# fanzhongyi/ExploreMultiModal

Measured on AMD Instinct MI355X. Metric: image-text pairs/sec fwd+bwd, VLMo-Base, 1/2/4/8 MI355X; % bf16 MFMA roofline, higher is better.
Workload: dtype bf16

## Files before the change

### exploremultimodal_amd/csrc/elementwise.hip

```cpp
#include "common.h"
#include "vlmo_hip.h"
#include <stdarg.h>
#include <stdio.h>

static thread_local char g_err[512] = "";
void vlmo_set_error(const char* fmt, ...) {
    va_list ap;
    va_start(ap, fmt);
    vsnprintf(g_err, sizeof(g_err), fmt, ap);
    va_end(ap);
}
extern "C" const char* vlmo_last_error(void) { return g_err; }
extern "C" int vlmo_abi_version(void) { return VLMO_ABI_VERSION; }

namespace {

__device__ __forceinline__ float fold_column(const float* __restrict__ ws, int ld, int ncols, int c, int r0, int r1) {
    float a = 0.f;
    if (c < ncols)
        for (int r = r0 + threadIdx.y; r < r1; r += 4) a += ws[(size_t)r * ld + c];
    return a;
}
template <typename T>
__device__ __forceinline__ void colsum8(const T* __restrict__ x, int ld, int ncols, int c8, int r0, int r1, float (&acc)[8]) {
// ... 308 lines not shown
        f32x4 g = *(const f32x4*)(dx + o);
        atype += g;
        if (thresh) {
            const uint64_t bits = drop_bits4(seed, o >> 2);
#pragma unroll
            for (int j = 0; j < 4; ++j) g[j] = drop_keep(bits, j, thresh) ? g[j] * inv_keep : 0.f;
        }
        apos += g;
        if (t > 0) {
            const bool mk = masked && masked[(size_t)b * npatch + t - 1];
            if (mk) amask += g;
            st4<bf16>(dproj + ((size_t)b * npatch + t - 1) * d + c4, mk ? f32x4{0.f, 0.f, 0.f, 0.f} : g);
        }
    }
#pragma unroll
    for (int j = 0; j < 4; ++j) {
        if (dpos) dpos[(size_t)t * d + c4 + j] += apos[j];
        if (dtype_row) atomicAdd(dtype_row + c4 + j, atype[j]);
        if (t == 0 && dcls) dcls[c4 + j] += apos[j];
        if (t > 0 && dmask && masked) atomicAdd(dmask + c4 + j, amask[j]);
    }
}

template <int VPL>
__device__ __forceinline__ void embed_txt_row(int64_t id, int t, int m, int lane, int nv, const float* __restrict__ word,
                                              const float* __restrict__ pos, const float* __restrict__ btype0,
                                              const float* __restrict__ ln_w, const float* __restrict__ ln_b,
                                              const float* __restrict__ type0, float* __restrict__ x,
                                              float* __restrict__ xhat, float* __restrict__ rstd, int d, float eps,
                                              uint32_t thresh, float inv_keep, uint64_t seed) {
    f32x4 v[VPL];
    float s = 0.f;
#pragma unroll
    for (int j = 0; j < VPL; ++j) {
        const int i = lane + 64 * j;
        if (i < nv) {
            v[j] = ((const f32x4*)(word + (size_t)id * d))[i] + ((const f32x4*)btype0)[i] +
                   ((const f32x4*)(pos + (size_t)t * d))[i];
            s += v[j][0] + v[j][1] + v[j][2] + v[j][3];
        } else {
            v[j] = f32x4{0.f, 0.f, 0.f, 0.f};
        }
    }
    const float mu = wave_sum(s) / d;
    float q = 0.f;
#pragma unroll
// ... 65 lines not shown
    }
    __device__ __forceinline__ void spill(float (*red)[VPL * 256], int lane) const {
#pragma unroll
        for (int j = 0; j < VPL; ++j)
#pragma unroll
            for (int k = 0; k < 4; ++k) {
                const int idx = (j * 64 + lane) * 4 + k;
                red[0][idx] = aw[j][k];
                red[1][idx] = ab[j][k];
                red[2][idx] = at[j][k];
                red[3][idx] = ae[j][k];
            }
    }
};

__device__ __forceinline__ int embed_txt_red_index(int c) {
    const int i = c >> 2;
    return ((i >> 6) * 64 + (i & 63)) * 4 + (c & 3);
}

template <int VPL>
__device__ __forceinline__ void embed_txt_row_bwd(int64_t id, int m, int lane, int nv, const float* __restrict__ dx,
                                                  const float* __restrict__ xhat, const float* __restrict__ rstd,
                                                  float* __restrict__ dword, EmbedTxtAcc<VPL>& A, int d, uint32_t thresh,
                                                  float inv_keep, uint64_t seed) {
    const float rs = rstd[m];
    f32x4 g[VPL], xh[VPL];
    float s1 = 0.f, s2 = 0.f;
#pragma unroll
    for (int j = 0; j < VPL; ++j) {
        const int i = lane + 64 * j;
        g[j] = f32x4{0.f, 0.f, 0.f, 0.f};
        xh[j] = g[j];
        if (i < nv) {
            f32x4 gy = ((const f32x4*)(dx + (size_t)m * d))[i];
            A.at[j] += gy;
            if (thresh) {
                const uint64_t bits = drop_bits4(seed, ((uint64_t)m * d >> 2) + i);
#pragma unroll
                for (int k = 0; k < 4; ++k) gy[k] = drop_keep(bits, k, thresh) ? gy[k] * inv_keep : 0.f;
            }
            xh[j] = ((const f32x4*)(xhat + (size_t)m * d))[i];
            A.aw[j] += gy * xh[j];
            A.ab[j] += gy;
            g[j] = gy * A.ww[j];
#pragma unroll
            for (int k = 0; k < 4; ++k) {
                s1 += g[j][k];
                s2 += g[j][k] * xh[j][k];
            }
        }
    }
    const float c1 = wave_sum(s1) / d, c2 = wave_sum(s2) / d;
#pragma unroll
    for (int j = 0; j < VPL; ++j) {
        const int i = lane + 64 * j;
        if (i < nv) {
            const f32x4 de = rs * (g[j] - c1 - xh[j] * c2);
            A.ae[j] += de;
#pragma unroll
            for (int k = 0; k < 4; ++k)
                if (dword && id != 0) atomicAdd(dword + (size_t)id * d + 4 * i + k, de[k]);
        }
    }
}

template <int VPL>
__global__ __launch_bounds__(256) void embed_txt_bwd_kernel(const float* __restrict__ dx, const int64_t* __restrict__ ids,
                                                            const float* __restrict__ xhat, const float* __restrict__ rstd,
                                                            const float* __restrict__ ln_w, float* __restrict__ dword,
                                                            float* __restrict__ dpos, float* __restrict__ dbtype0,
                                                            float* __restrict__ dln_w, float* __restrict__ dln_b,
                                                            float* __restrict__ dtype0, int ntok, int T, int d,
                                                            int rows_per_block, uint32_t thresh, float inv_keep,
                                                            uint64_t seed) {
    __shared__ float red[4][4][VPL * 256];
    const int lane = threadIdx.x & 63, wave = threadIdx.x >> 6, nv = d >> 2;
    EmbedTxtAcc<VPL> A;
    A.init(ln_w, lane, nv);
    const int t = blockIdx.x % T;
    const int b0 = (blockIdx.x / T) * rows_per_block, b1 = min(ntok / T, b0 + rows_per_block);
    for (int bq = b0 + wave; bq < b1; bq += 4) {
        const int m = bq * T + t;
        embed_txt_row_bwd<VPL>(ids[m], m, lane, nv, dx, xhat, rstd, dword, A, d, thresh, inv_keep, seed);
    }
    A.spill(red[wave], lane);
    __syncthreads();
    float* outs[4] = {dln_w, dln_b, dtype0, dbtype0};
    for (int c = threadIdx.x; c < d; c += 256) {
        const int idx = embed_txt_red_index(c);
#pragma unroll
        for (int w = 0; w < 4; ++w)
            if (outs[w]) atomicAdd(outs[w] + c, red[0][w][idx] + red[1][w][idx] + red[2][w][idx] + red[3][w][idx]);
        if (dpos) atomicAdd(dpos + (size_t)t * d + c, red[0][3][idx] + red[1][3][idx] + red[2][3][idx] + red[3][3][idx]);
    }
}

template <int VPL>
__global__ __launch_bounds__(256) void embed_txt_rows_bwd_kernel(const float* __restrict__ dx, const int64_t* __restrict__ ids,
                                                                 const int32_t* __restrict__ off, const float* __restrict__ xhat,
                                                                 const float* __restrict__ rstd, const float* __restrict__ ln_w,
                                                                 float* __restrict__ dword, float* __restrict__ ws, int B, int T,
                                                                 int maxlen, int d, int rows_per_block, uint32_t thresh,
                                                                 float inv_keep, uint64_t seed) {
    __shared__ float red[4][4][VPL * 256];
    const int lane = threadIdx.x & 63, wave = threadIdx.x >> 6, nv = d >> 2;
    EmbedTxtAcc<VPL> A;
    A.init(ln_w, lane, nv);
    const int t = blockIdx.x % maxlen;
    const int b0 = (blockIdx.x / maxlen) * rows_per_block, b1 = min(B, b0 + rows_per_block);
    for (int bq = b0 + wave; bq < b1; bq += 4) {
        const int r0 = off[bq];
        if (t >= off[bq + 1] - r0) continue;
        embed_txt_row_bwd<VPL>(ids[(size_t)bq * T + t], r0 + t, lane, nv, dx, xhat, rstd, dword, A, d, thresh, inv_keep,
                               seed);
    }
    A.spill(red[wave], lane);
    __syncthreads();
    float* row = ws + (size_t)blockIdx.x * 4 * d;
    for (int c = threadIdx.x; c < d; c += 256) {
        const int idx = embed_txt_red_index(c);
#pragma unroll
        for (int w = 0; w < 4; ++w) row[w * d + c] = red[0][w][idx] + red[1][w][idx] + red[2][w][idx] + red[3][w][idx];
    }
}

__global__ __launch_bounds__(256) void embed_txt_fold_kernel(const float* __restrict__ ws, int nrows, int maxlen, int d,
                                                             float* __restrict__ dln_w, float* __restrict__ dln_b,
                                                             float* __restrict__ dtype0, float* __restrict__ dbtype0,
                                                             float* __restrict__ dpos) {
    __shared__ float red[4][4][64];
    const int c = blockIdx.x * 64 + threadIdx.x, ld = 4 * d;
    if (blockIdx.y == 0) {
#pragma unroll
        for (int w = 0; w < 4; ++w) red[w][threadIdx.y][threadIdx.x] = fold_column(ws + w * d, ld, d, c, 0, nrows);
        __syncthreads();
        if (c < d) {
            const int w = threadIdx.y;
            float* out = w == 0 ? dln_w : (w == 1 ? dln_b : (w == 2 ? dtype0 : dbtype0));
            if (out) out[c] += red[w][0][threadIdx.x] + red[w][1][threadIdx.x] + red[w][2][threadIdx.x] + red[w][3][threadIdx.x];
        }
    } else {
        const int t = blockIdx.y - 1;
        red[0][threadIdx.y][threadIdx.x] = fold_column(ws + (size_t)t * ld + 3 * d, maxlen * ld, d, c, 0, nrows / maxlen);
        __syncthreads();
        if (threadIdx.y == 0 && c < d && dpos)
            dpos[(size_t)t * d + c] += red[0][0][threadIdx.x] + red[0][1][threadIdx.x] + red[0][2][threadIdx.x] + red[0][3][threadIdx.x];
    }
}

}

int fold_partials(const VlmoColJob& job, VlmoColJob* fold, hipStream_t stream) {
    if (fold) {
        *fold = job;
        return 0;
    }
    int slices = job.rows >= 64 ? 8 : 1;
    const int rps = (job.rows + slices - 1) / slices;
    slices = (job.rows + rps - 1) / rps;
    hipLaunchKernelGGL(reduce_partials_kernel, dim3((job.ncols + 63) / 64, slices), dim3(64, 4), 0, stream,
                       (const float*)job.src, job.rows, job.ncols, job.out[0], job.n0, job.out[1], rps, job.out[2], job.out[3]);
    VLMO_CHECK_LAUNCH("fold_partials");
    return 0;
}

extern "C" int64_t vlmo_reduce_ws_bytes(int ncols) { return reduce_ws_need(ncols); }

namespace {

// ... 145 lines not shown

extern "C" int vlmo_embed_img_finish(const void* proj, const float* cls_tok, const float* mask_tok, const float* pos,
                                     const float* type_row, const uint8_t* masked_pos, float* x, int B, int npatch,
                                     int d, uint32_t drop_thresh, float inv_keep, uint64_t seed, hipStream_t stream) {
    VLMO_CHECK_ARG(proj && cls_tok && mask_tok && pos && type_row && x, "vlmo_embed_img_finish: null pointer");
    VLMO_CHECK_ARG(B > 0 && npatch > 0 && d % 4 == 0 && d <= 4096, "vlmo_embed_img_finish: bad shape");
    hipLaunchKernelGGL(embed_img_finish_kernel, dim3(npatch + 1, B), dim3(d / 4), 0, stream, (const bf16*)proj, cls_tok,
                       mask_tok, pos, type_row, masked_pos, x, npatch, d, drop_thresh, inv_keep, seed);
    VLMO_CHECK_LAUNCH("vlmo_embed_img_finish");
    return 0;
}

extern "C" int vlmo_embed_img_bwd(const float* dx, const uint8_t* masked_pos, void* dproj, float* dcls, float* dmask,
                                  float* dpos, float* dtype_row, int B, int npatch, int d, uint32_t drop_thresh,
                                  float inv_keep, uint64_t seed, hipStream_t stream) {
    VLMO_CHECK_ARG(dx && dproj, "vlmo_embed_img_bwd: null pointer");
    VLMO_CHECK_ARG(B > 0 && npatch > 0 && d % 4 == 0 && d <= 4096, "vlmo_embed_img_bwd: bad shape");
    hipLaunchKernelGGL(embed_img_bwd_kernel, dim3(npatch + 1), dim3(d / 4), 0, stream, dx, masked_pos, (bf16*)dproj,
                       dcls, dmask, dpos, dtype_row, B, npatch, d, drop_thresh, inv_keep, seed);
    VLMO_CHECK_LAUNCH("vlmo_embed_img_bwd");
    return 0;
}

extern "C" int vlmo_embed_txt_fwd(const int64_t* ids, const float* word, const float* pos, const float* btype0,
                                  const float* ln_w, const float* ln_b, const float* type0, float* x, float* xhat,
                                  float* rstd, int B, int T, int d, float eps, uint32_t drop_thresh, float inv_keep,
                                  uint64_t seed, hipStream_t stream) {
    VLMO_CHECK_ARG(ids && word && pos && btype0 && ln_w && ln_b && type0 && x, "vlmo_embed_txt_fwd: null pointer");
    VLMO_CHECK_ARG(B > 0 && T > 0 && d % 4 == 0 && d <= 1024, "vlmo_embed_txt_fwd: bad shape");
    const int ntok = B * T;
    const int grid = (ntok + 3) / 4 < 8192 ? (ntok + 3) / 4 : 8192;
    dispatch_vpl(d, [&](auto V) {
        hipLaunchKernelGGL(embed_txt_fwd_kernel<decltype(V)::value>, dim3(grid), dim3(256), 0, stream, ids, word, pos, btype0,
                           ln_w, ln_b, type0, x, xhat, rstd, ntok, T, d, eps, drop_thresh, inv_keep, seed);
    });
    VLMO_CHECK_LAUNCH("vlmo_embed_txt_fwd");
    return 0;
}

extern "C" int vlmo_embed_txt_bwd(const float* dx, const int64_t* ids, const float* xhat, const float* rstd,
                                  const float* ln_w, float* dword, float* dpos, float* dbtype0, float* dln_w,
                                  float* dln_b, float* dtype0, int B, int T, int d, uint32_t drop_thresh,
                                  float inv_keep, uint64_t seed, hipStream_t stream) {
    VLMO_CHECK_ARG(dx && ids && xhat && rstd && ln_w, "vlmo_embed_txt_bwd: null pointer");
    VLMO_CHECK_ARG(B > 0 && T > 0 && d % 4 == 0 && d <= 1024, "vlmo_embed_txt_bwd: bad shape");
    const int ntok = B * T;
// ... 30 lines not shown
    if (B <= 0 || maxlen <= 0 || d <= 0) return 0;
    const int rpb = embed_txt_rows_rpb(B);
    return (int64_t)maxlen * ((B + rpb - 1) / rpb) * 4 * d * (int64_t)sizeof(float);
}

extern "C" int vlmo_embed_txt_rows_bwd(const float* dx, const int64_t* ids, const int32_t* off, const float* xhat,
                                       const float* rstd, const float* ln_w, float* dword, float* dpos, float* dbtype0,
                                       float* dln_w, float* dln_b, float* dtype0, float* ws, int64_t ws_bytes, int B, int T,
                                       int maxlen, int d, uint32_t drop_thresh, float inv_keep, uint64_t seed,
                                       hipStream_t stream) {
    VLMO_CHECK_ARG(dx && ids && off && xhat && rstd && ln_w && ws, "vlmo_embed_txt_rows_bwd: null pointer");
    VLMO_CHECK_ARG(B > 0 && T > 0 && maxlen > 0 && maxlen <= T && d % 4 == 0 && d > 0 && d <= 1024,
                   "vlmo_embed_txt_rows_bwd: bad shape B=%d T=%d maxlen=%d d=%d", B, T, maxlen, d);
    VLMO_CHECK_ARG(ws_bytes >= vlmo_embed_txt_rows_ws_bytes(B, maxlen, d),
                   "vlmo_embed_txt_rows_bwd: workspace too small (need %lld bytes)",
                   (long long)vlmo_embed_txt_rows_ws_bytes(B, maxlen, d));
    const int rpb = embed_txt_rows_rpb(B);
    const int grid = maxlen * ((B + rpb - 1) / rpb);
    dispatch_vpl(d, [&](auto V) {
        hipLaunchKernelGGL(embed_txt_rows_bwd_kernel<decltype(V)::value>, dim3(grid), dim3(256), 0, stream, dx, ids, off, xhat,
                           rstd, ln_w, dword, ws, B, T, maxlen, d, rpb, drop_thresh, inv_keep, seed);
    });
    VLMO_CHECK_LAUNCH("vlmo_embed_txt_rows_bwd");
    hipLaunchKernelGGL(embed_txt_fold_kernel, dim3((d + 63) / 64, 1 + maxlen), dim3(64, 4), 0, stream, (const float*)ws, grid,
                       maxlen, d, dln_w, dln_b, dtype0, dbtype0, dpos);
    VLMO_CHECK_LAUNCH("vlmo_embed_txt_rows_bwd");
    return 0;
}
```

### exploremultimodal_amd/engine.py

```python
import ctypes
import functools
import os as _os
import sys
from collections import namedtuple

import torch

from . import hip

LN_EPS = 1e-12
GRAD_SINK = None
_ov = _os.environ.get('VLMO_OVERLAP_WGRAD')
OVERLAP_WGRAD = None if _ov is None else _ov != '0'
ONE_STREAM_ROWS = 12288


def _use_side_stream(sink, rows):
    if OVERLAP_WGRAD is not None:
        return OVERLAP_WGRAD
    return sink is not None or rows < ONE_STREAM_ROWS


DEFAULT_TILE = -1

# ... 51 lines not shown

def _seg(a0, la, b0, lb, device):
    return torch.stack([a0, la, b0, lb], 1).to(device=device, dtype=torch.int32).contiguous()


class _PlanStatic:
    _cache = {}

    @classmethod
    def get(cls, B, T, P, device):
        key = (B, T, P, str(device))
        st = cls._cache.get(key)
        if st is None:
            st = cls(B, T, P, device)
            cls._cache[key] = st
        return st

    def __init__(self, B, T, P, device):
        nt = B * T
        ar = torch.arange(B, dtype=torch.int32)
        z = torch.zeros(B, dtype=torch.int32)
        tl, pl = torch.full((B,), T, dtype=torch.int32), torch.full((B,), P, dtype=torch.int32)
        self.seg_txt = _seg(ar * T, tl, z, z, device) if T else None
        self.seg_img = _seg(nt + ar * P, pl, z, z, device) if P else None
        self.seg_vl = _seg(ar * T, tl, nt + ar * P, pl, device) if (T and P) else None
        self.seg_sep = torch.cat([self.seg_img, self.seg_txt]).contiguous() if (T and P) else None
        N = T + P
        rm_t = (torch.arange(B).view(B, 1) * N + torch.arange(T).view(1, T)).reshape(-1)
        rm_i = (torch.arange(B).view(B, 1) * N + T + torch.arange(P).view(1, P)).reshape(-1)
        self.rowmap = torch.cat([rm_t, rm_i]).to(torch.int32).to(device)
        self.row_group = torch.cat([torch.arange(B).repeat_interleave(T),
                                    B + torch.arange(B).repeat_interleave(P)]).to(torch.int32).to(device)


def check_txt_lens(txt_lens, B, T):
    if torch.is_tensor(txt_lens):
        if txt_lens.device.type != 'cpu':
            raise ValueError('txt_lens must live on the host (python ints or a CPU tensor): reading a device tensor '
                             'would stall the pass (objectives.attach_text_lens builds it from the host batch)')
        if txt_lens.dim() != 1 or txt_lens.dtype.is_floating_point or txt_lens.dtype in (torch.bool, torch.complex64,
                                                                                          torch.complex128):
            raise ValueError(f'txt_lens must be a 1-D integer tensor, got {txt_lens.dtype} {tuple(txt_lens.shape)}')
        txt_lens = txt_lens.tolist()
    try:
        lens = tuple(txt_lens)
    except TypeError:
# ... 49 lines not shown
        self.seg_sep = torch.cat([self.seg_img, self.seg_txt]).contiguous() if P else None
        rb = torch.repeat_interleave(torch.arange(B, device=dev), ln.long(), output_size=nt)
        tt = torch.arange(nt, device=dev) - row0.long()[rb]
        self.src = (rb * T + tt).to(i32)
        N = T + P
        bi = torch.arange(B, device=dev).repeat_interleave(P)
        rm_i = bi * N + T + torch.arange(P, device=dev).repeat(B)
        self.rowmap = torch.cat([rb * N + tt, rm_i]).to(i32)
        self.row_group = torch.cat([rb, B + bi]).to(i32)


class Plan:

    def __init__(self, B, T, P, device, txt_mask=None, img_mask=None, txt_lens=None, txt_off=None):
        self.B, self.T, self.P = B, T, P
        self.device = device
        self.txt_lens = txt_lens
        if txt_lens is not None:
            assert T > 0
            st = _PlanRagged.get(B, T, P, device, txt_lens, txt_off)
            self.nt, self.maxT, self.txt_src, self.txt_off = st.nt, st.maxT, st.src, st.off
        else:
            st = _PlanStatic.get(B, T, P, device)
            self.nt, self.maxT = B * T, T
        self.ni = B * P
        self.M = self.nt + self.ni
        self.seg_txt, self.seg_img, self.seg_vl, self.seg_sep = st.seg_txt, st.seg_img, st.seg_vl, st.seg_sep
        self.rowmap, self.row_group = st.rowmap, st.row_group
        self.keymask = None
        if txt_mask is not None or img_mask is not None:
            txt, img = (m.reshape(-1).to(torch.int32) if n and m is not None else torch.ones(n, dtype=torch.int32, device=device)
                        for n, m in ((B * T, txt_mask), (self.ni, img_mask)))
            self.keymask = torch.cat([txt if txt_lens is None else txt[st.src.long()], img]).contiguous()

    def attn_launches(self, fused):
        if fused and self.seg_vl is not None:
            return [(self.seg_vl, self.B, self.maxT + self.P)]
        if self.seg_sep is not None:
            return [(self.seg_sep, 2 * self.B, max(self.maxT, self.P))]
        out = []
        if self.seg_txt is not None:
            out.append((self.seg_txt, self.B, self.maxT))
        if self.seg_img is not None:
            out.append((self.seg_img, self.B, self.P))
        return out


# ... 684 lines not shown
        pl, d, dev = meta['plan'], meta['d'], meta['device']
        B, T, P = pl.B, pl.T, pl.P
        drop, seed = meta['drop'], meta['seed']
        dx = dx.contiguous()
        g = [None] * 11
        npatch = P - 1 if P else 0
        shapes = [tuple(type_emb.shape)]
        if T:
            shapes += [tuple(word.shape), (meta['tpos_rows'], d), (2, d), (d,), (d,)]
        if P:
            shapes += [(d,), (d,), (P, d), (d, saved['img'].shape[1]), (d,)]
        sizes = [int(torch.Size(sh).numel()) for sh in shapes]
        flat = torch.zeros(sum(sizes), dtype=torch.float32, device=dev)
        views, o = [], 0
        for sh, n in zip(shapes, sizes):
            views.append(flat[o:o + n].view(sh))
            o += n
        dtype_emb = views[0]
        k = 1
        if T:
            xhat, rstd = saved['txt']
            dword, dtpos_full, dbtype, dlnw, dlnb = views[k:k + 5]
            k += 5
            if pl.txt_lens is None:
                hip.embed_txt_bwd(dx[:pl.nt], meta['ids'], xhat, rstd, ln_w, dword, dtpos_full[:T], dbtype[0], dlnw, dlnb,
                                  dtype_emb[0], B, T, d, drop=drop, seed=seed + 1)
            else:
                hip.embed_txt_rows_bwd(dx[:pl.nt], meta['ids'], pl.txt_off, xhat, rstd, ln_w, dword, dtpos_full[:T],
                                       dbtype[0], dlnw, dlnb, dtype_emb[0], B, T, pl.maxT, d, drop=drop, seed=seed + 1)
            g[6], g[7], g[8], g[9], g[10] = dword, dtpos_full, dbtype, dlnw, dlnb
        if P:
            patches = saved['img']
            dproj = torch.empty((B * npatch, d), dtype=torch.bfloat16, device=dev)
            dcls, dmask, dpos, dpw, dpb = views[k:k + 5]
            hip.embed_img_bwd(dx[pl.nt:], meta['masked'], dproj, dcls, dmask, dpos, dtype_emb[meta['img_type']],
                              B, npatch, d, drop=drop, seed=seed + 2)
            hip.gemm_tn(dproj, patches, dpw, B * npatch, d, patches.shape[1])
            hip.colsum(dproj, dpb, B * npatch, d)
            g[0], g[1] = dpw.view_as(patch_w), dpb
            g[2], g[4] = dcls, dpos
            g[3] = dmask if meta['masked'] is not None else None
        g[5] = dtype_emb
        return (None, *g)
```

### exploremultimodal_amd/hip.py

```python
import ctypes
import os

import numpy as np
import torch

_HERE = os.path.dirname(os.path.abspath(__file__))
LIB_PATH = os.environ.get('VLMO_HIP_LIB') or os.path.join(_HERE, 'lib', 'libvlmo_hip.so')

BF16, F16, F32 = 0, 1, 2
EPI_BIAS, EPI_BIAS_GELU, EPI_RESID, EPI_DGELU, EPI_F32, EPI_DUAL, EPI_ARGMAX, EPI_CE, EPI_CE_BWD = 0, 1, 2, 3, 4, 5, 6, 7, 8

_vp, _i32, _u32, _u64, _f32, _i64 = (ctypes.c_void_p, ctypes.c_int32, ctypes.c_uint32,
                                     ctypes.c_uint64, ctypes.c_float, ctypes.c_int64)


class Epilogue(ctypes.Structure):
    _fields_ = [('out', _vp), ('out2', _vp), ('bias', _vp), ('gamma', _vp),
                ('resid', _vp), ('row_scale', _vp), ('row_index', _vp), ('aux', _vp),
                ('ldo', _i32), ('ld2', _i32), ('relu', _i32),
                ('drop_thresh', _u32), ('inv_keep', _f32), ('beta', _f32),
                ('seed', _u64), ('colpart', _vp)]


_fp = _vp
# ... 56 lines not shown
_SIGS = {
    'vlmo_gemm_nt': [_i32, _i32, _i32, _vp, _i32, _vp, _i32, _i32, _i32, _i32,
                     ctypes.POINTER(Epilogue), _vp],
    'vlmo_gemm_tn': [_i32, _vp, _i32, _vp, _i32, _vp, _i32, _i32, _i32, _i32, _f32, _i32, _vp, _i64, _vp],
    'vlmo_ln_fwd': [_vp, _vp, _vp, _vp, _i32, _vp, _vp, _vp, _i32, _i32, _f32, _vp],
    'vlmo_ln_bwd': [_vp, _i32, _vp, _vp, _vp, _vp, _vp, _vp, _vp, _vp, _vp, _i32, _i32, _vp, _i64, _vp],
    'vlmo_ln_resid_bwd': [_vp, _vp, _vp, _vp, _vp, _vp, _vp, _vp, _vp, _vp, _vp, _vp, _vp, _vp, _vp, _vp, _u32, _f32, _u64,
                          _i32, _i32, _vp, _i64, _vp],
    'vlmo_attn_fwd': [_vp, _vp, _i32, _vp, _vp, _vp, _i32, _i32, _i32, _i32, _f32, _u32, _f32,
                      _u64, _i32, _vp],
    'vlmo_attn_bwd': [_vp, _vp, _vp, _vp, _i32, _vp, _i32, _vp, _vp, _vp, _i32, _i32, _i32, _f32,
                      _u32, _f32, _u64, _i32, _vp],
    'vlmo_attn_probs': [_vp, _vp, _i32, _vp, _vp, _i32, _i32, _i32, _i32, _i32, _i32, _f32, _vp],
    'vlmo_attn_gradcam': [_vp, _vp, _vp, _i32, _vp, _vp, _i32, _i32, _i32, _i32, _i32, _i32, _i32, _f32, _vp],
    'vlmo_resid_bwd': [_vp, _vp, _vp, _vp, _vp, _vp, _vp, _vp, _i32, _i32, _u32, _f32, _u64, _vp, _i64, _vp],
    'vlmo_colsum': [_i32, _vp, _i32, _vp, _i32, _i32, _vp, _i64, _vp],
    'vlmo_cast_weight': [_i32, _vp, _i32, _i32, _vp, _vp, _vp],
    'vlmo_cast_weight_multi': [_i32, _i32, _vp, _vp, _vp, _vp, _vp, _vp],
    'vlmo_patchify': [_vp, _vp, _i32, _i32, _i32, _i32, _i32, _vp],
    'vlmo_embed_img_finish': [_vp, _vp, _vp, _vp, _vp, _vp, _vp, _i32, _i32, _i32, _u32, _f32,
                              _u64, _vp],
    'vlmo_embed_img_bwd': [_vp, _vp, _vp, _vp, _vp, _vp, _vp, _i32, _i32, _i32, _u32, _f32,
                           _u64, _vp],
    'vlmo_embed_txt_fwd': [_vp] * 10 + [_i32, _i32, _i32, _f32, _u32, _f32, _u64, _vp],
    'vlmo_embed_txt_bwd': [_vp] * 11 + [_i32, _i32, _i32, _u32, _f32, _u64, _vp],
    'vlmo_embed_txt_rows_fwd': [_vp] * 11 + [_i32, _i32, _i32, _f32, _u32, _f32, _u64, _vp],
    'vlmo_embed_txt_rows_bwd': [_vp] * 13 + [_i64, _i32, _i32, _i32, _i32, _u32, _f32, _u64, _vp],
    'vlmo_conv2d_nhwc': [_i32, _i32, _vp, _i32, _i32, _i32, _i32, _i32, _vp, _i32, _vp,
                         ctypes.POINTER(Epilogue), _vp],
    'vlmo_dvae_im2col': [_vp, _vp, _i32, _i32, _i32, _i32, _i32, _i32, _vp],
    'vlmo_maxpool2_nhwc': [_vp, _vp, _vp, _i32, _i32, _i32, _i32, _vp],
    'vlmo_argmax_reduce': [_vp, _i32, _vp, _i32, _vp],
    'vlmo_dvae_embed': [_vp, _vp, _vp, _vp, _i32, _i32, _i32, _vp],
    'vlmo_upsample2_nhwc': [_vp, _vp, _i32, _i32, _i32, _i32, _vp],
    'vlmo_dvae_out_head': [_vp, _vp, _vp, _vp, _i32, _i32, _i32, _i32, _i32, _vp],
    'vlmo_conv4s2_nhwc': [_i32, _vp, _i32, _i32, _i32, _i32, _vp, _i32, _vp, ctypes.POINTER(Epilogue), _vp],
    'vlmo_convt4s2_nhwc': [_i32, _vp, _i32, _i32, _i32, _i32, _vp, _i32, _vp, ctypes.POINTER(Epilogue), _vp],
    'vlmo_dvae_patch4s2': [_vp, _vp, _i32, _i32, _i32, _i32, _i32, _vp],
    'vlmo_dvae_out_head_linear': [_vp, _vp, _vp, _vp, _i32, _i32, _i32, _i32, _i32, _vp],
    'vlmo_ce_reduce': [_vp, _i32, _vp, _i32, _vp, _vp, _vp, _i32, _vp],
    'vlmo_stack_fwd': [ctypes.POINTER(StackDesc), _vp],
    'vlmo_stack_bwd': [ctypes.POINTER(StackDesc), _vp],
    'vlmo_gemm_tn_multi': [_i32, ctypes.POINTER(TnProblem), _i32, _vp],
    'vlmo_gemm_tn_multi_plan': [ctypes.POINTER(TnProblem), _i32, ctypes.POINTER(_i32), ctypes.POINTER(_i32),
                                ctypes.POINTER(TnProblemPlan), ctypes.POINTER(_i32), ctypes.POINTER(ctypes.c_uint16)],
    'vlmo_colwork_multi': [_i32, ctypes.POINTER(ColJob), _i32, _vp],
# ... 15 lines not shown
    'vlmo_comm_unique_id': [_vp],
    'vlmo_comm_init': [ctypes.POINTER(ctypes.c_void_p), _vp, _i32, _i32],
    'vlmo_comm_destroy': [_vp],
    'vlmo_comm_count': [_vp, _vp, _vp],
    'vlmo_comm_all_reduce': [_vp, _vp, _vp, _i64, _i32, _vp],
    'vlmo_comm_reduce_scatter': [_vp, _vp, _vp, _i64, _i32, _vp],
    'vlmo_comm_all_gather': [_vp, _vp, _vp, _i64, _i32, _vp],
    'vlmo_grad_pack': [_vp, _vp, _i64, _f32, _vp],
    'vlmo_grad_unpack': [_vp, _vp, _i64, _vp],
    'vlmo_ln_gelu_fwd': [_vp, _i32, _vp, _vp, _vp, _i32, _vp, _vp, _i32, _i32, _f32, _vp],
    'vlmo_ln_gelu_bwd': [_vp, _i32, _vp, _i32, _vp, _vp, _vp, _vp, _vp, _i32, _vp, _i32, _vp, _vp, _vp, _i32, _i32, _vp,
                         _i64, _vp],
    'vlmo_vqa_bce': [_vp, _i32, _vp, _i32, _i32, _i32, _vp, _vp, _vp, _vp, _f32, _vp, _i32, _vp, _i32, _vp],
    'vlmo_isda_update': [_vp, _i32, _vp, _vp, _vp, _vp, _vp, _i32, _i32, _i32, _i32, _vp, _vp, _vp, _vp, _vp],
    'vlmo_isda_aug_fwd': [_vp, _i32, _vp, _vp, _i32, _i32, _i32, _i32, _f32, _vp, _i32, _vp, _i64, _vp],
    'vlmo_isda_aug_bwd': [_vp, _i32, _vp, _i32, _vp, _vp, _i32, _i32, _i32, _i32, _f32, _vp, _i32, _vp, _i64, _vp],
    'vlmo_sim_topk': [_vp, _i32, _vp, _i32, _i32, _i32, _i32, _i32, _f32, _i32, _vp, ctypes.c_size_t, _vp, _vp, _vp],
    'vlmo_crop_resample': [_vp, _i64, _vp, _vp, _i32, _vp, _vp, _i32, ctypes.POINTER(_f32), ctypes.POINTER(_f32), _f32, _vp,
                           _i64, _vp],
    'vlmo_randaug': [_vp, _vp, _vp, _i64, _vp, _vp, _i32, _vp, _vp, _i32, _i32, _vp, _i64, _vp],
}

_lib = None
ABI_VERSION = 16

def lib():
    global _lib
    if _lib is None:
        if not os.path.exists(LIB_PATH):
            raise RuntimeError(
                f'{LIB_PATH} not found: build the HIP extension first '
                '(python -c "import __graft_entry__ as g; g.build()" or '
                'make -C exploremultimodal_amd/csrc). There is no CPU fallback.')
        L = ctypes.CDLL(LIB_PATH)
        L.vlmo_last_error.restype = ctypes.c_char_p
        L.vlmo_abi_version.restype = ctypes.c_int
        if L.vlmo_abi_version() != ABI_VERSION:
            raise RuntimeError(f'{LIB_PATH} has ABI version {L.vlmo_abi_version()}, this package needs {ABI_VERSION}: '
                               'rebuild it (make -C exploremultimodal_amd/csrc)')
        L.vlmo_reduce_ws_bytes.restype = ctypes.c_int64
        L.vlmo_reduce_ws_bytes.argtypes = [_i32]
        L.vlmo_stack_bwd_ws_bytes.restype = ctypes.c_int64
        L.vlmo_stack_bwd_ws_bytes.argtypes = [_i32, _i32, _i32, _i32]
        L.vlmo_gemm_tn_ws_bytes.restype = ctypes.c_int64
        L.vlmo_isda_ws_bytes.restype = ctypes.c_int64
        L.vlmo_isda_ws_bytes.argtypes = [_i32, _i32, _i32]
        L.vlmo_gemm_tn_ws_bytes.argtypes = [_i32, _i32, _i32]
        L.vlmo_sim_topk_ws_bytes.restype = ctypes.c_int64
        L.vlmo_sim_topk_ws_bytes.argtypes = [_i32, _i32, _i32, _i32]
        L.vlmo_randaug_ws_bytes.restype = ctypes.c_int64
        L.vlmo_randaug_ws_bytes.argtypes = [_i32]
        L.vlmo_embed_txt_rows_ws_bytes.restype = ctypes.c_int64
        L.vlmo_embed_txt_rows_ws_bytes.argtypes = [_i32, _i32, _i32]
        for name, sig in _SIGS.items():
            fn = getattr(L, name)
            fn.argtypes = sig
            fn.restype = ctypes.c_int
        _lib = L
    return _lib


def exported_symbols():
    return ['vlmo_last_error', 'vlmo_abi_version', 'vlmo_reduce_ws_bytes', 'vlmo_stack_bwd_ws_bytes',
            'vlmo_gemm_tn_ws_bytes', 'vlmo_isda_ws_bytes', 'vlmo_sim_topk_ws_bytes', 'vlmo_randaug_ws_bytes',
            'vlmo_embed_txt_rows_ws_bytes'] + list(_SIGS)


def _check(rc, name):
    if rc != 0:
        raise RuntimeError(f'{name} failed (rc={rc}): {lib().vlmo_last_error().decode()}')


def _p(t):
    return None if t is None else t.data_ptr()


def _stream():
    return torch.cuda.current_stream().cuda_stream


def _dt(t):
    return {torch.bfloat16: BF16, torch.float16: F16, torch.float32: F32}[t.dtype]


_SCRATCH = {}


def _scratch(kind, device, nbytes, floor):
# ... 156 lines not shown

def patchify(img, out, patch):
    B, C, H, W = img.shape
    rc = lib().vlmo_patchify(_p(img), _p(out), B, C, H, W, patch, _stream())
    _check(rc, 'vlmo_patchify')


def embed_img_finish(proj, cls_tok, mask_tok, pos, type_row, masked, x, B, npatch, d,
                     drop=(0, 1.0), seed=0):
    rc = lib().vlmo_embed_img_finish(_p(proj), _p(cls_tok), _p(mask_tok), _p(pos), _p(type_row),
                                     _p(masked), _p(x), B, npatch, d, drop[0], drop[1],
                                     _seed64(seed), _stream())
    _check(rc, 'vlmo_embed_img_finish')


def embed_img_bwd(dx, masked, dproj, dcls, dmask, dpos, dtype_row, B, npatch, d, drop=(0, 1.0),
                  seed=0):
    rc = lib().vlmo_embed_img_bwd(_p(dx), _p(masked), _p(dproj), _p(dcls), _p(dmask), _p(dpos),
                                  _p(dtype_row), B, npatch, d, drop[0], drop[1],
                                  _seed64(seed), _stream())
    _check(rc, 'vlmo_embed_img_bwd')


def embed_txt_fwd(ids, word, pos, btype0, ln_w, ln_b, type0, x, xhat, rstd, B, T, d, eps,
                  drop=(0, 1.0), seed=0):
    rc = lib().vlmo_embed_txt_fwd(_p(ids), _p(word), _p(pos), _p(btype0), _p(ln_w), _p(ln_b),
                                  _p(type0), _p(x), _p(xhat), _p(rstd), B, T, d, eps, drop[0],
                                  drop[1], _seed64(seed), _stream())
    _check(rc, 'vlmo_embed_txt_fwd')


def embed_txt_bwd(dx, ids, xhat, rstd, ln_w, dword, dpos, dbtype0, dln_w, dln_b, dtype0, B, T, d,
                  drop=(0, 1.0), seed=0):
    rc = lib().vlmo_embed_txt_bwd(_p(dx), _p(ids), _p(xhat), _p(rstd), _p(ln_w), _p(dword),
                                  _p(dpos), _p(dbtype0), _p(dln_w), _p(dln_b), _p(dtype0), B, T, d,
                                  drop[0], drop[1], _seed64(seed), _stream())
    _check(rc, 'vlmo_embed_txt_bwd')


def embed_txt_rows_fwd(ids, src, word, pos, btype0, ln_w, ln_b, type0, x, xhat, rstd, nrows, T, d, eps,
                       drop=(0, 1.0), seed=0):
    rc = lib().vlmo_embed_txt_rows_fwd(_p(ids), _p(src), _p(word), _p(pos), _p(btype0), _p(ln_w), _p(ln_b),
                                       _p(type0), _p(x), _p(xhat), _p(rstd), nrows, T, d, eps, drop[0],
                                       drop[1], _seed64(seed), _stream())
    _check(rc, 'vlmo_embed_txt_rows_fwd')


def embed_txt_rows_bwd(dx, ids, off, xhat, rstd, ln_w, dword, dpos, dbtype0, dln_w, dln_b, dtype0, B, T, maxlen, d,
                       drop=(0, 1.0), seed=0):
    nbytes = lib().vlmo_embed_txt_rows_ws_bytes(B, maxlen, d)
    ws = _scratch('embed_txt_rows', dx.device, nbytes, 1 << 20)
    rc = lib().vlmo_embed_txt_rows_bwd(_p(dx), _p(ids), _p(off), _p(xhat), _p(rstd), _p(ln_w), _p(dword),
                                       _p(dpos), _p(dbtype0), _p(dln_w), _p(dln_b), _p(dtype0), _p(ws),
                                       ws.numel() * 4, B, T, maxlen, d, drop[0], drop[1], _seed64(seed), _stream())
    _check(rc, 'vlmo_embed_txt_rows_bwd')


_ZERO = {}


def zero_page(device):
    z = _ZERO.get(device)
    if z is None:
        z = torch.zeros(256, dtype=torch.float32, device=device)
        _ZERO[device] = z
    return z


def conv2d_nhwc(epi, x, B, H, W, Cin, kw, w, Cout, out, *, out2=None, bias=None, resid=None, relu=False,
                relu_in=False, beta=0.0, ldo=None):
    e = _epilogue(out, out2=out2, bias=bias, resid=resid, relu=int(relu) | (2 if relu_in else 0), beta=beta, ldo=ldo)
    rc = lib().vlmo_conv2d_nhwc(epi, _dt(x), _p(x), B, H, W, Cin, kw, _p(w), Cout, _p(zero_page(x.device)),
                                ctypes.byref(e), _stream())
    _check(rc, 'vlmo_conv2d_nhwc')
# ... 382 lines not shown
```

### include/vlmo_hip.h

```cpp
#ifndef VLMO_HIP_H
#define VLMO_HIP_H

#include <stddef.h>
#include <stdint.h>

#ifdef __cplusplus
extern "C" {
#endif

#ifndef __HIP_PLATFORM_AMD__
typedef struct ihipStream_t* hipStream_t;
#endif

enum { VLMO_BF16 = 0, VLMO_F16 = 1, VLMO_F32 = 2 };

enum {
    VLMO_EPI_BIAS = 0,
    VLMO_EPI_BIAS_GELU = 1,
    VLMO_EPI_RESID = 2,
    VLMO_EPI_DGELU = 3,
    VLMO_EPI_F32 = 4,
    VLMO_EPI_DUAL = 5,
    VLMO_EPI_ARGMAX = 6,
    VLMO_EPI_CE = 7,
    VLMO_EPI_CE_BWD = 8
};

typedef struct VlmoEpilogue {
    void* out;
    void* out2;
    const float* bias;
    const float* gamma;
    const float* resid;
    const float* row_scale;
    const int32_t* row_index;
    const void* aux;
    int32_t ldo, ld2;
    int32_t relu;
    uint32_t drop_thresh;
    float inv_keep;
    float beta;
    uint64_t seed;
    float* colpart;
} VlmoEpilogue;

const char* vlmo_last_error(void);
#define VLMO_ABI_VERSION 16
int vlmo_abi_version(void);

int vlmo_gemm_nt(int epi, int dtype, int tile, const void* A, int lda, const void* B, int ldb,
                 int M, int N, int K, const VlmoEpilogue* e, hipStream_t stream);
int vlmo_gemm_nt_2src(int epi, int dtype, int tile, const void* A, int lda, int k1, float seg_scale, const void* A2,
                      int lda2, const void* B, int ldb, int M, int N, int K, const VlmoEpilogue* e,
                      hipStream_t stream);
int vlmo_gemm_nt_grouped(int epi, int dtype, int tile, int ngroups, const void* const* A, int lda,
                         const void* const* B, int ldb, const int32_t* M, int N, int K,
                         const VlmoEpilogue* e, hipStream_t stream);

int64_t vlmo_gemm_tn_ws_bytes(int M, int N1, int N2);
int vlmo_gemm_tn(int dtype, const void* A, int lda, const void* B, int ldb, float* C, int ldc,
                 int M, int N1, int N2, float alpha, int splits, float* ws, int64_t ws_bytes,
                 hipStream_t stream);

typedef struct VlmoTnProblem {
    const void* A;
    const void* B;
    float* C;
    int32_t lda, ldb, ldc;
    int32_t M, N1, N2;
    float alpha;
// ... 55 lines not shown
typedef struct VlmoColJob {
    int32_t kind, ld;
    const void* src;
    int32_t rows, ncols;
    float* out[4];
    int32_t n0, pad_;
} VlmoColJob;
int vlmo_colwork_multi(int dtype, const VlmoColJob* jobs, int n, hipStream_t stream);

int vlmo_cast_weight(int dtype, const float* src, int rows, int cols, void* dst, void* dstT,
                     hipStream_t stream);
int vlmo_cast_weight_multi(int dtype, int n, const float* const* src, const int32_t* rows, const int32_t* cols,
                           void* const* dst, void* const* dstT, hipStream_t stream);

int vlmo_patchify(const float* img, void* out, int B, int C, int H, int W, int patch,
                  hipStream_t stream);
int vlmo_embed_img_finish(const void* proj, const float* cls_tok, const float* mask_tok,
                          const float* pos, const float* type_row, const uint8_t* masked_pos,
                          float* x, int B, int npatch, int d, uint32_t drop_thresh,
                          float inv_keep, uint64_t seed, hipStream_t stream);
int vlmo_embed_img_bwd(const float* dx, const uint8_t* masked_pos, void* dproj, float* dcls,
                       float* dmask, float* dpos, float* dtype_row, int B, int npatch, int d,
                       uint32_t drop_thresh, float inv_keep, uint64_t seed, hipStream_t stream);

int vlmo_embed_txt_fwd(const int64_t* ids, const float* word, const float* pos, const float* btype0,
                       const float* ln_w, const float* ln_b, const float* type0, float* x,
                       float* xhat, float* rstd, int B, int T, int d, float eps,
                       uint32_t drop_thresh, float inv_keep, uint64_t seed, hipStream_t stream);
int vlmo_embed_txt_bwd(const float* dx, const int64_t* ids, const float* xhat, const float* rstd,
                       const float* ln_w, float* dword, float* dpos, float* dbtype0, float* dln_w,
                       float* dln_b, float* dtype0, int B, int T, int d, uint32_t drop_thresh,
                       float inv_keep, uint64_t seed, hipStream_t stream);
int vlmo_embed_txt_rows_fwd(const int64_t* ids, const int32_t* src, const float* word, const float* pos,
                            const float* btype0, const float* ln_w, const float* ln_b, const float* type0,
                            float* x, float* xhat, float* rstd, int nrows, int T, int d, float eps,
                            uint32_t drop_thresh, float inv_keep, uint64_t seed, hipStream_t stream);
int64_t vlmo_embed_txt_rows_ws_bytes(int B, int maxlen, int d);
int vlmo_embed_txt_rows_bwd(const float* dx, const int64_t* ids, const int32_t* off, const float* xhat,
                            const float* rstd, const float* ln_w, float* dword, float* dpos, float* dbtype0,
                            float* dln_w, float* dln_b, float* dtype0, float* ws, int64_t ws_bytes, int B, int T,
                            int maxlen, int d, uint32_t drop_thresh, float inv_keep, uint64_t seed,
                            hipStream_t stream);

int vlmo_profile_start(int max_records);
int vlmo_profile_stop(int ntags, double* ms, double* flops, int64_t* launches);

// ... 199 lines not shown
```

Before: 4619.

## Split embedding backward over batch chunks with workspace fold; coalesce word-grad atomics

```diff
diff --git a/exploremultimodal_amd/csrc/elementwise.hip b/exploremultimodal_amd/csrc/elementwise.hip
--- a/exploremultimodal_amd/csrc/elementwise.hip
+++ b/exploremultimodal_amd/csrc/elementwise.hip
@@ -354,6 +354,95 @@
     }
 }
 
+__global__ void embed_img_bwd_ws_kernel(const float* __restrict__ dx, const uint8_t* __restrict__ masked,
+                                        bf16* __restrict__ dproj, float* __restrict__ ws, int B, int npatch, int d, int cs,
+                                        uint32_t thresh, float inv_keep, uint64_t seed) {
+    const int t = blockIdx.x, c4 = threadIdx.x * 4;
+    const int b0 = blockIdx.y * cs, b1 = min(B, b0 + cs);
+    f32x4 apos = {0.f, 0.f, 0.f, 0.f}, atype = apos, amask = apos;
+    for (int bb = b0; bb < b1; bb += 4) {
+        f32x4 gk[4];
+        bool mkk[4];
+#pragma unroll
+        for (int k = 0; k < 4; ++k) {
+            const int b = min(bb + k, b1 - 1);
+            gk[k] = *(const f32x4*)(dx + ((size_t)b * (npatch + 1) + t) * d + c4);
+            mkk[k] = t > 0 && masked && masked[(size_t)b * npatch + t - 1];
+        }
+#pragma unroll
+        for (int k = 0; k < 4; ++k) {
+            const int b = bb + k;
+            if (b >= b1) break;
+            const size_t o = ((size_t)b * (npatch + 1) + t) * d + c4;
+            f32x4 g = gk[k];
+            atype += g;
+            if (thresh) {
+                const uint64_t bits = drop_bits4(seed, o >> 2);
+#pragma unroll
+                for (int j = 0; j < 4; ++j) g[j] = drop_keep(bits, j, thresh) ? g[j] * inv_keep : 0.f;
+            }
+            apos += g;
+            if (t > 0) {
+                if (mkk[k]) amask += g;
+                st4<bf16>(dproj + ((size_t)b * npatch + t - 1) * d + c4, mkk[k] ? f32x4{0.f, 0.f, 0.f, 0.f} : g);
+            }
+        }
+    }
+    float* row = ws + ((size_t)blockIdx.y * (npatch + 1) + t) * 3 * d + c4;
+    *(f32x4*)row = apos;
+    *(f32x4*)(row + d) = atype;
+    if (masked) *(f32x4*)(row + 2 * d) = amask;
+}
+
+struct EmbedFold {
+    const float* ws;
+    int nchunks, P, d, nparts, pos_part;
+    float* all[4];
+    float *dpos, *dcls;
+};
+__global__ __launch_bounds__(1024) void embed_fold_kernel(const EmbedFold f) {
+    __shared__ float red[16][64];
+    const int c = blockIdx.x * 64 + threadIdx.x, d = f.d, P = f.P;
+    const size_t ld = (size_t)f.nparts * d;
+    if ((int)blockIdx.y < f.nparts) {
+        float* out = f.all[blockIdx.y];
+        if (!out) return;
+        const float* src = f.ws + (size_t)blockIdx.y * d;
+        const int nrows = f.nchunks * P;
+        float a = 0.f;
+        if (c < d)
+            for (int r = threadIdx.y; r < nrows; r += 64) {
+                float v[4];
+#pragma unroll
+                for (int k = 0; k < 4; ++k) v[k] = r + 16 * k < nrows ? src[(r + 16 * k) * ld + c] : 0.f;
+#pragma unroll
+                for (int k = 0; k < 4; ++k) a += v[k];
+            }
+        red[threadIdx.y][threadIdx.x] = a;
+        __syncthreads();
+        if (threadIdx.y == 0 && c < d) {
+            float s = red[0][threadIdx.x];
+#pragma unroll
+            for (int y = 1; y < 16; ++y) s += red[y][threadIdx.x];
+            out[c] += s;
+        }
+    } else {
+        const int t = ((int)blockIdx.y - f.nparts) * 16 + threadIdx.y;
+        if (t < P && c < d) {
+            const float* src = f.ws + (size_t)f.pos_part * d + c;
+            float a = src[t * ld];
+            for (int k = 1; k < f.nchunks; ++k) a += src[((size_t)k * P + t) * ld];
+            if (f.dpos) f.dpos[(size_t)t * d + c] += a;
+            if (t == 0 && f.dcls) f.dcls[c] += a;
+        }
+    }
+}
+int embed_fold_launch(const EmbedFold& f, hipStream_t stream) {
+    hipLaunchKernelGGL(embed_fold_kernel, dim3((f.d + 63) / 64, f.nparts + (f.P + 15) / 16), dim3(64, 16), 0, stream, f);
+    VLMO_CHECK_LAUNCH("embed_fold");
+    return 0;
+}
+
 template <int VPL>
 __device__ __forceinline__ void embed_txt_row(int64_t id, int t, int m, int lane, int nv, const float* __restrict__ word,
                                               const float* __restrict__ pos, const float* __restrict__ btype0,
@@ -465,9 +554,10 @@
 template <int VPL>
 __device__ __forceinline__ void embed_txt_row_bwd(int64_t id, int m, int lane, int nv, const float* __restrict__ dx,
                                                   const float* __restrict__ xhat, const float* __restrict__ rstd,
-                                                  float* __restrict__ dword, EmbedTxtAcc<VPL>& A, int d, uint32_t thresh,
-                                                  float inv_keep, uint64_t seed) {
+                                                  float* __restrict__ dword, EmbedTxtAcc<VPL>& A, float* xp, int d,
+                                                  uint32_t thresh, float inv_keep, uint64_t seed) {
     const float rs = rstd[m];
+    const bool scatter = dword && id != 0;
     f32x4 g[VPL], xh[VPL];
     float s1 = 0.f, s2 = 0.f;
 #pragma unroll
@@ -501,10 +591,21 @@
         if (i < nv) {
             const f32x4 de = rs * (g[j] - c1 - xh[j] * c2);
             A.ae[j] += de;
-#pragma unroll
-            for (int k = 0; k < 4; ++k)
-                if (dword && id != 0) atomicAdd(dword + (size_t)id * d + 4 * i + k, de[k]);
-        }
+            if (scatter) ((f32x4*)xp)[i] = de;
+        }
+    }
+    if (scatter) {
+        __builtin_amdgcn_fence(__ATOMIC_RELEASE, "wavefront");
+        __builtin_amdgcn_wave_barrier();
+        __builtin_amdgcn_fence(__ATOMIC_ACQUIRE, "wavefront");
+        float* wrow = dword + (size_t)id * d;
+#pragma unroll
+        for (int q = 0; q < 4 * VPL; ++q) {
+            const int c = lane + 64 * q;
+            if (c < d) atomicAdd(wrow + c, xp[c]);
+        }
+        __builtin_amdgcn_fence(__ATOMIC_RELEASE, "wavefront");
+        __builtin_amdgcn_wave_barrier();
     }
 }
 
@@ -525,7 +626,7 @@
     const int b0 = (blockIdx.x / T) * rows_per_block, b1 = min(ntok / T, b0 + rows_per_block);
     for (int bq = b0 + wave; bq < b1; bq += 4) {
         const int m = bq * T + t;
-        embed_txt_row_bwd<VPL>(ids[m], m, lane, nv, dx, xhat, rstd, dword, A, d, thresh, inv_keep, seed);
+        embed_txt_row_bwd<VPL>(ids[m], m, lane, nv, dx, xhat, rstd, dword, A, red[wave][0], d, thresh, inv_keep, seed);
     }
     A.spill(red[wave], lane);
     __syncthreads();
@@ -555,8 +656,8 @@
     for (int bq = b0 + wave; bq < b1; bq += 4) {
         const int r0 = off[bq];
         if (t >= off[bq + 1] - r0) continue;
-        embed_txt_row_bwd<VPL>(ids[(size_t)bq * T + t], r0 + t, lane, nv, dx, xhat, rstd, dword, A, d, thresh, inv_keep,
-                               seed);
+        embed_txt_row_bwd<VPL>(ids[(size_t)bq * T + t], r0 + t, lane, nv, dx, xhat, rstd, dword, A, red[wave][0], d, thresh,
+                               inv_keep, seed);
     }
     A.spill(red[wave], lane);
     __syncthreads();
@@ -565,30 +666,6 @@
         const int idx = embed_txt_red_index(c);
 #pragma unroll
         for (int w = 0; w < 4; ++w) row[w * d + c] = red[0][w][idx] + red[1][w][idx] + red[2][w][idx] + red[3][w][idx];
-    }
-}
-
-__global__ __launch_bounds__(256) void embed_txt_fold_kernel(const float* __restrict__ ws, int nrows, int maxlen, int d,
-                                                             float* __restrict__ dln_w, float* __restrict__ dln_b,
-                                                             float* __restrict__ dtype0, float* __restrict__ dbtype0,
-                                                             float* __restrict__ dpos) {
-    __shared__ float red[4][4][64];
-    const int c = blockIdx.x * 64 + threadIdx.x, ld = 4 * d;
-    if (blockIdx.y == 0) {
-#pragma unroll
-        for (int w = 0; w < 4; ++w) red[w][threadIdx.y][threadIdx.x] = fold_column(ws + w * d, ld, d, c, 0, nrows);
-        __syncthreads();
-        if (c < d) {
-            const int w = threadIdx.y;
-            float* out = w == 0 ? dln_w : (w == 1 ? dln_b : (w == 2 ? dtype0 : dbtype0));
-            if (out) out[c] += red[w][0][threadIdx.x] + red[w][1][threadIdx.x] + red[w][2][threadIdx.x] + red[w][3][threadIdx.x];
-        }
-    } else {
-        const int t = blockIdx.y - 1;
-        red[0][threadIdx.y][threadIdx.x] = fold_column(ws + (size_t)t * ld + 3 * d, maxlen * ld, d, c, 0, nrows / maxlen);
-        __syncthreads();
-        if (threadIdx.y == 0 && c < d && dpos)
-            dpos[(size_t)t * d + c] += red[0][0][threadIdx.x] + red[0][1][threadIdx.x] + red[0][2][threadIdx.x] + red[0][3][threadIdx.x];
     }
 }
 
@@ -780,6 +857,39 @@
     return 0;
 }
 
+namespace {
+int embed_img_chunk(int B, int npatch, int d) {
+    const int per_chunk = (npatch + 1) * ((d / 4 + 63) / 64);
+    const int want = (8 * 256 + per_chunk - 1) / per_chunk;
+    const int cs = (B + want - 1) / want;
+    return cs < 4 ? 4 : cs;
+}
+}
+
+extern "C" int64_t vlmo_embed_img_bwd_ws_bytes(int B, int npatch, int d) {
+    if (B <= 0 || npatch <= 0 || d <= 0) return 0;
+    const int cs = embed_img_chunk(B, npatch, d);
+    return (int64_t)((B + cs - 1) / cs) * (npatch + 1) * 3 * d * (int64_t)sizeof(float);
+}
+
+extern "C" int vlmo_embed_img_bwd_ws(const float* dx, const uint8_t* masked_pos, void* dproj, float* dcls, float* dmask,
+                                     float* dpos, float* dtype_row, float* ws, int64_t ws_bytes, int B, int npatch, int d,
+                                     uint32_t drop_thresh, float inv_keep, uint64_t seed, hipStream_t stream) {
+    VLMO_CHECK_ARG(dx && dproj && ws, "vlmo_embed_img_bwd_ws: null pointer");
+    VLMO_CHECK_ARG(B > 0 && npatch > 0 && d > 0 && d % 4 == 0 && d <= 4096, "vlmo_embed_img_bwd_ws: bad shape");
+    VLMO_CHECK_ARG(ws_bytes >= vlmo_embed_img_bwd_ws_bytes(B, npatch, d),
+                   "vlmo_embed_img_bwd_ws: workspace too small (need %lld bytes)",
+                   (long long)vlmo_embed_img_bwd_ws_bytes(B, npatch, d));
+    const int cs = embed_img_chunk(B, npatch, d);
+    const int chunks = (B + cs - 1) / cs;
+    VLMO_CHECK_ARG(chunks <= 65535, "vlmo_embed_img_bwd_ws: batch too large");
+    hipLaunchKernelGGL(embed_img_bwd_ws_kernel, dim3(npatch + 1, chunks), dim3(d / 4), 0, stream, dx, masked_pos,
+                       (bf16*)dproj, ws, B, npatch, d, cs, drop_thresh, inv_keep, seed);
+    VLMO_CHECK_LAUNCH("vlmo_embed_img_bwd_ws");
+    return embed_fold_launch(EmbedFold{ws, chunks, npatch + 1, d, 3, 0, {nullptr, dtype_row, masked_pos ? dmask : nullptr, nullptr},
+                                       dpos, dcls}, stream);
+}
+
 extern "C" int vlmo_embed_txt_fwd(const int64_t* ids, const float* word, const float* pos, const float* btype0,
                                   const float* ln_w, const float* ln_b, const float* type0, float* x, float* xhat,
                                   float* rstd, int B, int T, int d, float eps, uint32_t drop_thresh, float inv_keep,
@@ -856,8 +966,5 @@
                            rstd, ln_w, dword, ws, B, T, maxlen, d, rpb, drop_thresh, inv_keep, seed);
     });
     VLMO_CHECK_LAUNCH("vlmo_embed_txt_rows_bwd");
-    hipLaunchKernelGGL(embed_txt_fold_kernel, dim3((d + 63) / 64, 1 + maxlen), dim3(64, 4), 0, stream, (const float*)ws, grid,
-                       maxlen, d, dln_w, dln_b, dtype0, dbtype0, dpos);
-    VLMO_CHECK_LAUNCH("vlmo_embed_txt_rows_bwd");
-    return 0;
-}
+    return embed_fold_launch(EmbedFold{ws, grid / maxlen, maxlen, d, 4, 3, {dln_w, dln_b, dtype0, dbtype0}, dpos, nullptr}, stream);
+}
diff --git a/exploremultimodal_amd/engine.py b/exploremultimodal_amd/engine.py
--- a/exploremultimodal_amd/engine.py
+++ b/exploremultimodal_amd/engine.py
@@ -97,6 +97,7 @@
         z = torch.zeros(B, dtype=torch.int32)
         tl, pl = torch.full((B,), T, dtype=torch.int32), torch.full((B,), P, dtype=torch.int32)
         self.seg_txt = _seg(ar * T, tl, z, z, device) if T else None
+        self.txt_off = (torch.arange(B + 1, dtype=torch.int32) * T).to(device) if T else None
         self.seg_img = _seg(nt + ar * P, pl, z, z, device) if P else None
         self.seg_vl = _seg(ar * T, tl, nt + ar * P, pl, device) if (T and P) else None
         self.seg_sep = torch.cat([self.seg_img, self.seg_txt]).contiguous() if (T and P) else None
@@ -192,7 +193,7 @@
             self.nt, self.maxT, self.txt_src, self.txt_off = st.nt, st.maxT, st.src, st.off
         else:
             st = _PlanStatic.get(B, T, P, device)
-            self.nt, self.maxT = B * T, T
+            self.nt, self.maxT, self.txt_off = B * T, T, st.txt_off
         self.ni = B * P
         self.M = self.nt + self.ni
         self.seg_txt, self.seg_img, self.seg_vl, self.seg_sep = st.seg_txt, st.seg_img, st.seg_vl, st.seg_sep
@@ -923,19 +924,17 @@
             xhat, rstd = saved['txt']
             dword, dtpos_full, dbtype, dlnw, dlnb = views[k:k + 5]
             k += 5
-            if pl.txt_lens is None:
-                hip.embed_txt_bwd(dx[:pl.nt], meta['ids'], xhat, rstd, ln_w, dword, dtpos_full[:T], dbtype[0], dlnw, dlnb,
-                                  dtype_emb[0], B, T, d, drop=drop, seed=seed + 1)
-            else:
-                hip.embed_txt_rows_bwd(dx[:pl.nt], meta['ids'], pl.txt_off, xhat, rstd, ln_w, dword, dtpos_full[:T],
-                                       dbtype[0], dlnw, dlnb, dtype_emb[0], B, T, pl.maxT, d, drop=drop, seed=seed + 1)
+            ws = _persist(dev, 'embed_txt_ws', hip.embed_txt_rows_ws_bytes(B, pl.maxT, d) // 4, torch.float32)
+            hip.embed_txt_rows_bwd(dx[:pl.nt], meta['ids'], pl.txt_off, xhat, rstd, ln_w, dword, dtpos_full[:T],
+                                   dbtype[0], dlnw, dlnb, dtype_emb[0], B, T, pl.maxT, d, drop=drop, seed=seed + 1, ws=ws)
             g[6], g[7], g[8], g[9], g[10] = dword, dtpos_full, dbtype, dlnw, dlnb
         if P:
             patches = saved['img']
             dproj = torch.empty((B * npatch, d), dtype=torch.bfloat16, device=dev)
             dcls, dmask, dpos, dpw, dpb = views[k:k + 5]
-            hip.embed_img_bwd(dx[pl.nt:], meta['masked'], dproj, dcls, dmask, dpos, dtype_emb[meta['img_type']],
-                              B, npatch, d, drop=drop, seed=seed + 2)
+            ws = _persist(dev, 'embed_img_ws', hip.embed_img_bwd_ws_bytes(B, npatch, d) // 4, torch.float32)
+            hip.embed_img_bwd_ws(dx[pl.nt:], meta['masked'], dproj, dcls, dmask, dpos, dtype_emb[meta['img_type']],
+                                 B, npatch, d, drop=drop, seed=seed + 2, ws=ws)
             hip.gemm_tn(dproj, patches, dpw, B * npatch, d, patches.shape[1])
             hip.colsum(dproj, dpb, B * npatch, d)
             g[0], g[1] = dpw.view_as(patch_w), dpb
diff --git a/exploremultimodal_amd/hip.py b/exploremultimodal_amd/hip.py
--- a/exploremultimodal_amd/hip.py
+++ b/exploremultimodal_amd/hip.py
@@ -102,6 +102,7 @@
                               _u64, _vp],
     'vlmo_embed_img_bwd': [_vp, _vp, _vp, _vp, _vp, _vp, _vp, _i32, _i32, _i32, _u32, _f32,
                            _u64, _vp],
+    'vlmo_embed_img_bwd_ws': [_vp] * 8 + [_i64, _i32, _i32, _i32, _u32, _f32, _u64, _vp],
     'vlmo_embed_txt_fwd': [_vp] * 10 + [_i32, _i32, _i32, _f32, _u32, _f32, _u64, _vp],
     'vlmo_embed_txt_bwd': [_vp] * 11 + [_i32, _i32, _i32, _u32, _f32, _u64, _vp],
     'vlmo_embed_txt_rows_fwd': [_vp] * 11 + [_i32, _i32, _i32, _f32, _u32, _f32, _u64, _vp],
@@ -163,7 +164,7 @@
 }
 
 _lib = None
-ABI_VERSION = 16
+ABI_VERSION = 17
 
 def lib():
     global _lib
@@ -193,6 +194,8 @@
         L.vlmo_randaug_ws_bytes.argtypes = [_i32]
         L.vlmo_embed_txt_rows_ws_bytes.restype = ctypes.c_int64
         L.vlmo_embed_txt_rows_ws_bytes.argtypes = [_i32, _i32, _i32]
+        L.vlmo_embed_img_bwd_ws_bytes.restype = ctypes.c_int64
+        L.vlmo_embed_img_bwd_ws_bytes.argtypes = [_i32, _i32, _i32]
         for name, sig in _SIGS.items():
             fn = getattr(L, name)
             fn.argtypes = sig
@@ -204,7 +207,7 @@
 def exported_symbols():
     return ['vlmo_last_error', 'vlmo_abi_version', 'vlmo_reduce_ws_bytes', 'vlmo_stack_bwd_ws_bytes',
             'vlmo_gemm_tn_ws_bytes', 'vlmo_isda_ws_bytes', 'vlmo_sim_topk_ws_bytes', 'vlmo_randaug_ws_bytes',
-            'vlmo_embed_txt_rows_ws_bytes'] + list(_SIGS)
+            'vlmo_embed_txt_rows_ws_bytes', 'vlmo_embed_img_bwd_ws_bytes'] + list(_SIGS)
 
 
 def _check(rc, name):
@@ -407,6 +410,18 @@
     _check(rc, 'vlmo_embed_img_bwd')
 
 
+def embed_img_bwd_ws_bytes(B, npatch, d):
+    return lib().vlmo_embed_img_bwd_ws_bytes(B, npatch, d)
+
+
+def embed_img_bwd_ws(dx, masked, dproj, dcls, dmask, dpos, dtype_row, B, npatch, d, drop=(0, 1.0), seed=0, ws=None):
+    if ws is None:
+        ws = _scratch('embed_img_bwd', dx.device, embed_img_bwd_ws_bytes(B, npatch, d), 1 << 20)
+    rc = lib().vlmo_embed_img_bwd_ws(_p(dx), _p(masked), _p(dproj), _p(dcls), _p(dmask), _p(dpos), _p(dtype_row),
+                                     _p(ws), ws.numel() * 4, B, npatch, d, drop[0], drop[1], _seed64(seed), _stream())
+    _check(rc, 'vlmo_embed_img_bwd_ws')
+
+
 def embed_txt_fwd(ids, word, pos, btype0, ln_w, ln_b, type0, x, xhat, rstd, B, T, d, eps,
                   drop=(0, 1.0), seed=0):
     rc = lib().vlmo_embed_txt_fwd(_p(ids), _p(word), _p(pos), _p(btype0), _p(ln_w), _p(ln_b),
@@ -431,10 +446,14 @@
     _check(rc, 'vlmo_embed_txt_rows_fwd')
 
 
+def embed_txt_rows_ws_bytes(B, maxlen, d):
+    return lib().vlmo_embed_txt_rows_ws_bytes(B, maxlen, d)
+
+
 def embed_txt_rows_bwd(dx, ids, off, xhat, rstd, ln_w, dword, dpos, dbtype0, dln_w, dln_b, dtype0, B, T, maxlen, d,
-                       drop=(0, 1.0), seed=0):
-    nbytes = lib().vlmo_embed_txt_rows_ws_bytes(B, maxlen, d)
-    ws = _scratch('embed_txt_rows', dx.device, nbytes, 1 << 20)
+                       drop=(0, 1.0), seed=0, ws=None):
+    if ws is None:
+        ws = _scratch('embed_txt_rows', dx.device, embed_txt_rows_ws_bytes(B, maxlen, d), 1 << 20)
     rc = lib().vlmo_embed_txt_rows_bwd(_p(dx), _p(ids), _p(off), _p(xhat), _p(rstd), _p(ln_w), _p(dword),
                                        _p(dpos), _p(dbtype0), _p(dln_w), _p(dln_b), _p(dtype0), _p(ws),
                                        ws.numel() * 4, B, T, maxlen, d, drop[0], drop[1], _seed64(seed), _stream())
diff --git a/include/vlmo_hip.h b/include/vlmo_hip.h
--- a/include/vlmo_hip.h
+++ b/include/vlmo_hip.h
@@ -45,7 +45,7 @@
 } VlmoEpilogue;
 
 const char* vlmo_last_error(void);
-#define VLMO_ABI_VERSION 16
+#define VLMO_ABI_VERSION 17
 int vlmo_abi_version(void);
 
 int vlmo_gemm_nt(int epi, int dtype, int tile, const void* A, int lda, const void* B, int ldb,
@@ -147,6 +147,11 @@
 int vlmo_embed_img_bwd(const float* dx, const uint8_t* masked_pos, void* dproj, float* dcls,
                        float* dmask, float* dpos, float* dtype_row, int B, int npatch, int d,
                        uint32_t drop_thresh, float inv_keep, uint64_t seed, hipStream_t stream);
+int64_t vlmo_embed_img_bwd_ws_bytes(int B, int npatch, int d);
+int vlmo_embed_img_bwd_ws(const float* dx, const uint8_t* masked_pos, void* dproj, float* dcls,
+                          float* dmask, float* dpos, float* dtype_row, float* ws, int64_t ws_bytes,
+                          int B, int npatch, int d, uint32_t drop_thresh, float inv_keep, uint64_t seed,
+                          hipStream_t stream);
 
 int vlmo_embed_txt_fwd(const int64_t* ids, const float* word, const float* pos, const float* btype0,
                        const float* ln_w, const float* ln_b, const float* type0, float* x,
```

Result: no change. 4639 (median of 6 runs) (+0.4%).
